# shehryar-malik/icrl

Hardware: AMD Instinct MI355X
Metric: env-steps/sec (ICRL outer loop, HCWithPos-v0) (higher is better)
Workload: dtype f32

## Files before the change

icrl_amd/csrc/rollout.hip:

```cpp
#include <stdio.h>
#include <stdlib.h>

#include "common.h"
#include "cost_fn.h"
#include "generic.h"

namespace icrl {

__global__ void policy_transpose_kernel(PolLayout L, const float* __restrict__ p, float* __restrict__ pt) {
  for (int i = blockIdx.x * blockDim.x + threadIdx.x; i < L.n; i += gridDim.x * blockDim.x) {
    int dst = i;
    for (int w = 0; w < 3; ++w) {
      if (i >= L.W1[w] && i < L.b1[w]) { int r = i - L.W1[w]; int j = r / L.O, k = r % L.O; dst = L.W1[w] + k * L.H1 + j; }
      if (i >= L.W2[w] && i < L.b2[w]) { int r = i - L.W2[w]; int j = r / L.H1, k = r % L.H1; dst = L.W2[w] + k * L.H2 + j; }
    }
    if (i >= L.Wa && i < L.ba) { int r = i - L.Wa; int a = r / L.H2, j = r % L.H2; dst = L.Wa + j * L.A + a; }
    pt[dst] = p[i];
  }
}

__global__ void costnet_transpose_kernel(CnLayout L, const float* __restrict__ p, float* __restrict__ pt) {
  for (int i = blockIdx.x * blockDim.x + threadIdx.x; i < L.n; i += gridDim.x * blockDim.x) {
    int dst = i;
    if (i >= L.W0 && i < L.b0) { int r = i - L.W0; int j = r / L.in, k = r % L.in; dst = L.W0 + k * L.H1 + j; }
    if (L.nh == 2 && i >= L.W1 && i < L.b1) { int r = i - L.W1; int j = r / L.H1, k = r % L.H1; dst = L.W1 + k * L.H2 + j; }
    pt[dst] = p[i];
  }
}

typedef float f32x4 __attribute__((ext_vector_type(4)));

struct ActShared {
  alignas(16) double s_old[MAX_OBS];
  alignas(16) double s_new[MAX_OBS];
  alignas(16) float x[MAX_OBS];
  alignas(16) float h[3][MAX_H];
  alignas(16) float g[3][MAX_H];
  alignas(16) float cx[MAX_CN_IN];
  alignas(16) float ch[2][MAX_H];
  float act_raw[MAX_ACT];
  float act_clip[MAX_ACT];
  float scal[4];
};

template <int OCT, int CIT>
struct WaveRegs {
  static constexpr int NA = 16 * (OCT > CIT ? OCT : CIT);
  union { float w1[NA]; float c0[NA]; };
  union { float w2[MAX_H]; float c1[MAX_H]; };
  float wh[MAX_H];
  union { float b1; float cb0; };
  union { float b2; float cb1; };
  union { float bh; float cbo; };
  union { float ls; float co; };
  float sd, lsd, i2v;
  int sel[(16 * (CIT > 0 ? CIT : 1) + WAVE - 1) / WAVE];
};
template <int OCT> using PolRegs = WaveRegs<OCT, 0>;
template <int CIT> using CnRegs = WaveRegs<0, CIT>;

template <int OCT, class Regs>
__device__ __forceinline__ void load_pol_regs(const PolLayout& L, const float* __restrict__ PT, Regs& R) {
  const int lane = threadIdx.x & 63;
  const int w = __builtin_amdgcn_readfirstlane(threadIdx.x >> 6);
  const int j1 = lane < L.H1 ? lane : 0, j2 = lane < L.H2 ? lane : 0;
#pragma unroll
  for (int k = 0; k < 16 * OCT; ++k) R.w1[k] = (w < 3 && k < L.O) ? PT[L.W1[w] + k * L.H1 + j1] : 0.f;
#pragma unroll
  for (int k = 0; k < MAX_H; ++k) R.w2[k] = (w < 3 && k < L.H1) ? PT[L.W2[w] + k * L.H2 + j2] : 0.f;
  R.b1 = w < 3 ? PT[L.b1[w] + j1] : 0.f;
  R.b2 = w < 3 ? PT[L.b2[w] + j2] : 0.f;
  R.bh = 0.f; R.ls = 0.f; R.sd = 1.f; R.lsd = 0.f; R.i2v = 2.f;
  if (w == 0) {
    const int a = lane < L.A ? lane : 0;
#pragma unroll
    for (int j = 0; j < MAX_H; ++j) R.wh[j] = j < L.H2 ? PT[L.Wa + j * L.A + a] : 0.f;
    R.bh = PT[L.ba + a];
    if (!L.discrete) R.ls = PT[L.log_std + a];
    R.sd = expf(R.ls); R.lsd = logf(R.sd); R.i2v = 2.f * (R.sd * R.sd);
  } else if (w < 3) {
#pragma unroll
    for (int j = 1; j < MAX_H; ++j) R.wh[j] = 0.f;
    R.wh[0] = PT[(w == 1 ? L.Wv : L.Wc) + j2];
    R.bh = PT[w == 1 ? L.bv : L.bc];
  }
}

template <int OCT, class Regs>
__device__ __forceinline__ void policy_forward_block(const PolLayout& L, const Regs& R, ActShared& sh,
                                                     const float* noise_row, int deterministic,
                                                     const float* alow, const float* ahigh,
                                                     const float* given = nullptr ) {
  const int lane = threadIdx.x & 63;
  const int w = __builtin_amdgcn_readfirstlane(threadIdx.x >> 6);
  if (w < 3) {
    f32x4 xs[4 * OCT];
#pragma unroll
    for (int i = 0; i < 4 * OCT; ++i) xs[i] = *reinterpret_cast<const f32x4*>(&sh.x[4 * i]);
    float acc = 0.f;
#pragma unroll
    for (int k = 0; k < 16 * OCT; ++k) acc = fmaf(R.w1[k], xs[k >> 2][k & 3], acc);
    sh.h[w][lane] = lane < L.H1 ? fast_tanh(acc + R.b1) : 0.f;
  }
  __syncthreads();
  if (w < 3) {
    f32x4 hs[MAX_H / 4];
#pragma unroll
    for (int i = 0; i < MAX_H / 4; ++i) hs[i] = *reinterpret_cast<const f32x4*>(&sh.h[w][4 * i]);
    float acc = 0.f;
#pragma unroll
    for (int k = 0; k < MAX_H; ++k) acc = fmaf(R.w2[k], hs[k >> 2][k & 3], acc);
    sh.g[w][lane] = lane < L.H2 ? fast_tanh(acc + R.b2) : 0.f;
  }
  __syncthreads();
  if (w == 0) {
    float mean = 0.f;
    {
      f32x4 gs[MAX_H / 4];
#pragma unroll
      for (int i = 0; i < MAX_H / 4; ++i) gs[i] = *reinterpret_cast<const f32x4*>(&sh.g[0][4 * i]);
      float acc = 0.f;
#pragma unroll
      for (int j = 0; j < MAX_H; ++j) acc = fmaf(R.wh[j], gs[j >> 2][j & 3], acc);
      mean = acc + R.bh;
    }
    if (!L.discrete) {
      float lp = 0.f, entl = 0.f;
      if (lane < L.A) {
        const float std = R.sd;
        float act = mean;
        if (given != nullptr) act = given[lane];
        else if (!deterministic) act = mean + noise_row[lane] * std;
        const float diff = act - mean;
        lp = -(diff * diff) / R.i2v - R.lsd - LOG_SQRT_2PI_F;
        entl = HALF_LOG_2PI_PLUS_HALF_F + R.lsd;
        sh.act_raw[lane] = act;
        float c = act;
        if (alow != nullptr && ahigh != nullptr) c = fminf(fmaxf(act, alow[lane]), ahigh[lane]);
        sh.act_clip[lane] = c;
      }
      lp = wave_sum_fast(lp);
      const float ent = wave_sum_fast(entl);
      if (lane == 0) { sh.scal[2] = lp; sh.scal[3] = ent; }
    } else {
      float m = wave_max(lane < L.A ? mean : -INFINITY);
      float e = lane < L.A ? expf(mean - m) : 0.f;
      float lse = m + logf(wave_sum(e));
      float logp = mean - lse;
      float p = lane < L.A ? expf(logp) : 0.f;
      float cdf = 0.f;
      int action = 0;
      if (given != nullptr) {
        action = (int)given[0];
      } else if (deterministic) {
        float best = wave_max(lane < L.A ? p : -1.f);
        unsigned long long ball = __ballot(lane < L.A && p == best);
        action = __ffsll((long long)ball) - 1;
      } else {
        const float u = noise_row[0];
        int cnt = 0;
        for (int a = 0; a < L.A; ++a) {
          cdf += __shfl(p, a, 64);
          cnt += (u >= cdf) ? 1 : 0;
        }
        action = cnt < L.A - 1 ? cnt : L.A - 1;
      }
      const float lp = __shfl(logp, action, 64);
      const float ent = -wave_sum(lane < L.A ? logp * p : 0.f);
      if (lane == 0) { sh.scal[2] = lp; sh.scal[3] = ent; sh.act_raw[0] = (float)action; sh.act_clip[0] = (float)action; }
    }
  } else if (w < 3) {
    float part = lane < L.H2 ? R.wh[0] * sh.g[w][lane] : 0.f;
    part = wave_sum_fast(part);
    if (lane == 0) sh.scal[w - 1] = part + R.bh;
  }
}

template <int CIT, class Regs>
__device__ __forceinline__ void load_cn_regs(const icrl_costnet_t& cn, const CnLayout& L, Regs& R) {
  const int lane = threadIdx.x & 63;
  const float* PT = cn.params_t;
  const int j1 = lane < L.H1 ? lane : 0, j2 = lane < L.H2 ? lane : 0;
#pragma unroll
  for (int k = 0; k < 16 * CIT; ++k) R.c0[k] = k < L.in ? PT[L.W0 + k * L.H1 + j1] : 0.f;
#pragma unroll
  for (int k = 0; k < MAX_H; ++k) R.c1[k] = (L.nh == 2 && k < L.H1) ? PT[L.W1 + k * L.H2 + j2] : 0.f;
  R.cb0 = PT[L.b0 + j1];
  R.cb1 = L.nh == 2 ? PT[L.b1 + j2] : 0.f;
  R.co = PT[L.Wo + j2];
  R.cbo = PT[L.bo];
#pragma unroll
  for (int i = 0; i < (16 * CIT + WAVE - 1) / WAVE; ++i) { const int idx = lane + i * WAVE; R.sel[i] = idx < L.in ? cn.select_dim[idx] : -1; }
}

template <int CIT, class Regs>
__device__ __forceinline__ float cost_forward_wave(const icrl_costnet_t& cn, const CnLayout& L, const Regs& R,
                                                   const double* obs_row, const float* acs_row, float* cx, float (*ch)[MAX_H],
                                                   int mode = 0 ) {
  const int lane = threadIdx.x & 63;
#pragma unroll
  for (int i = 0; i < (16 * CIT + WAVE - 1) / WAVE; ++i) {
    const int idx = lane + i * WAVE;
    const int sel = R.sel[i];
    float v = 0.f;
    if (sel >= 0) {
      if (sel < cn.obs_dim) {
        double o = obs_row[sel];
        if (cn.obs_mean != nullptr && cn.obs_var != nullptr) o = (o - cn.obs_mean[sel]) / sqrt(cn.obs_var[sel] + cn.eps);
        if (cn.clip_obs >= 0.0) o = fmin(fmax(o, -cn.clip_obs), cn.clip_obs);
        v = (float)o;
      } else {
        const int a = sel - cn.obs_dim;
        float x;
        if (cn.is_discrete) x = ((int)acs_row[0] == a) ? 1.f : 0.f;
        else x = acs_row[a];
        if (cn.action_low != nullptr && cn.action_high != nullptr) x = fminf(fmaxf(x, cn.action_low[a]), cn.action_high[a]);
        v = x;
      }
    }
    if (idx < 16 * CIT) cx[idx] = v;
  }
  __builtin_amdgcn_wave_barrier();
  __builtin_amdgcn_s_waitcnt(0xC07F);
  {
    f32x4 xs[4 * CIT];
#pragma unroll
    for (int i = 0; i < 4 * CIT; ++i) xs[i] = *reinterpret_cast<const f32x4*>(&cx[4 * i]);
    float acc = 0.f;
#pragma unroll
    for (int k = 0; k < 16 * CIT; ++k) acc = fmaf(R.c0[k], xs[k >> 2][k & 3], acc);
    ch[0][lane] = lane < L.H1 ? fmaxf(acc + R.cb0, 0.f) : 0.f;
  }
  __builtin_amdgcn_wave_barrier();
  __builtin_amdgcn_s_waitcnt(0xC07F);
  int last = 0;
  if (L.nh == 2) {
    f32x4 hs[MAX_H / 4];
#pragma unroll
    for (int i = 0; i < MAX_H / 4; ++i) hs[i] = *reinterpret_cast<const f32x4*>(&ch[0][4 * i]);
    float acc = 0.f;
#pragma unroll
    for (int k = 0; k < MAX_H; ++k) acc = fmaf(R.c1[k], hs[k >> 2][k & 3], acc);
    ch[1][lane] = lane < L.H2 ? fmaxf(acc + R.cb1, 0.f) : 0.f;
    __builtin_amdgcn_wave_barrier();
    __builtin_amdgcn_s_waitcnt(0xC07F);
    last = 1;
  }
  float part = lane < L.H2 ? R.co * ch[last][lane] : 0.f;
  const float z = wave_sum_fast(part) + R.cbo;
  const float zeta = 1.f / (1.f + expf(-z));
  if (mode == 1) return zeta;
  if (mode == 2) return logf(zeta + (float)cn.eps);
  return 1.f - zeta;
}

template <bool POINT = true>
__device__ __forceinline__ double env_reset_value(const icrl_env_t& e, uint32_t key, uint32_t ctr, int i) {
  if (POINT && e.reward_form >= 4) return e.reward_form == 12 ? (i == 0 ? 3.0 : 5.0) : 0.0;
  if (e.reward_form >= 2) return -1.0;
  return (unit_uniform(key, ctr, (uint32_t)(e.obs_dim + i)) - 0.5) * 0.2;
}

__device__ __forceinline__ void lap_grid_step_wave(const icrl_env_t& e, int n, const double* s_old, const float* act,
                                                   uint32_t& ctr_io, int& tep_io, double* s_new_lds, double& reward,
                                                   int& done) {
  const int lane = threadIdx.x & 63;
  const int pos_old = (int)llrint((s_old[0] + 1.0) * 20.0);
  const int ac = (int)act[0];
  int pos = pos_old, d = 0;
  double rew;
  if (ac == 0) {
    pos = pos_old + 1 == 40 ? 0 : pos_old + 1;
    rew = (pos % 10 == 5) ? 3.0 : 0.0;
  } else if (e.reward_form == 3) {
    rew = -1.0;
    d = 1;
  } else {
    pos = pos_old == 0 ? 39 : pos_old - 1;
    rew = (pos % 10 == 5) ? 3.0 : 0.0;
  }
  const int tep = tep_io + 1;
  if (tep >= e.max_steps) d = 1;
  if (d) pos = 0;
  const double v = ((double)pos * 2.0) / 40.0 - 1.0;
  tep_io = d ? 0 : tep;
  ctr_io = ctr_io + 1u;
  if (lane == 0) {
    e.s[n] = v;
    if (s_new_lds != nullptr) s_new_lds[0] = v;
    e.t_ep[n] = tep_io;
    e.step_count[n] = ctr_io;
  }
  reward = rew;
  done = d;
}

struct PointStep { double rew; int done; };
__device__ __forceinline__ int bridge_orientation(double p0, double p1, double q0, double q1, double r0, double r1) {
  const double val = ((q1 - p1) * (r0 - q0)) - ((q0 - p0) * (r1 - q1));
  return val == 0.0 ? 0 : (val > 0.0 ? 1 : -1);
}
__device__ __forceinline__ bool bridge_on_segment(double p0, double p1, double q0, double q1, double r0, double r1) {
  return r0 <= fmax(p0, q0) && r0 >= fmin(p0, q0) && r1 <= fmax(p1, q1) && r1 >= fmin(p1, q1);
}
__device__ __forceinline__ bool bridge_in_region(double sx, double sy, double nx, double ny, double ox, double oy, double w, double h) {
  const double x1 = ox + w, y1 = oy + h;
  if (sx > ox && sx < x1 && sy > oy && sy < y1) return true;
  if (nx > ox && nx < x1 && ny > oy && ny < y1) return true;
  bool hit = false;
#pragma unroll 1
  for (int b = 0; b < 4; ++b) {
    const double bp0 = b == 2 ? x1 : ox, bp1 = b == 3 ? y1 : oy;
    const double bq0 = b == 1 ? ox : x1, bq1 = b == 0 ? oy : y1;
    const int o1 = bridge_orientation(sx, sy, nx, ny, bp0, bp1);
    const int o2 = bridge_orientation(sx, sy, nx, ny, bq0, bq1);
    const int o3 = bridge_orientation(bp0, bp1, bq0, bq1, sx, sy);
    const int o4 = bridge_orientation(bp0, bp1, bq0, bq1, nx, ny);
    if (o1 != o2 && o3 != o4) hit = true;
    if (o1 == 0 && bridge_on_segment(sx, sy, nx, ny, bp0, bp1)) hit = true;
    if (o2 == 0 && bridge_on_segment(sx, sy, nx, ny, bq0, bq1)) hit = true;
    if (o3 == 0 && bridge_on_segment(bp0, bp1, bq0, bq1, sx, sy)) hit = true;
    if (o4 == 0 && bridge_on_segment(bp0, bp1, bq0, bq1, nx, ny)) hit = true;
  }
  return hit;
}
__device__ __noinline__ PointStep bridge_step_wave(int form, int max_steps, double* s_all, int32_t* t_ep_all, uint32_t* step_count_all,
                                                   int n, double x0, double y0, double ori0, float act0, float act1, uint32_t ctr_new,
                                                   int tep, double* s_new_lds) {
  const int lane = threadIdx.x & 63;
  const bool cont = form >= 13;
// ... 636 lines not shown
#pragma unroll
    for (int k = 0; k < 16; ++k) { const double d = va[k] - bm; va[k] = d * d; }
    __builtin_amdgcn_sched_barrier(0);
#pragma unroll
    for (int k = 0; k < 16; ++k) if (r0 + k < N) sq += va[k];
    load16(r0 + 32 < N ? r0 + 32 : 0, va);
#pragma unroll
    for (int k = 0; k < 16; ++k) { const double d = vb[k] - bm; vb[k] = d * d; }
    __builtin_amdgcn_sched_barrier(0);
#pragma unroll
    for (int k = 0; k < 16; ++k) if (r0 + 16 + k < N) sq += vb[k];
  }
  bv = sq / (double)N;
}

__device__ __forceinline__ void column_moments_contig(const double* col, int N, double& bm, double& bv) {
  double va[16], vb[16];
  double sum = 0.0;
  const int NF = N & ~31;
#pragma unroll
  for (int k = 0; k < 16; ++k) va[k] = col[k];
  int r0 = 0;
  for (; r0 < NF; r0 += 32) {
#pragma unroll
    for (int k = 0; k < 16; ++k) vb[k] = col[r0 + 16 + k];
    __builtin_amdgcn_sched_barrier(0);
#pragma unroll
    for (int k = 0; k < 16; ++k) sum += va[k];
#pragma unroll
    for (int k = 0; k < 16; ++k) va[k] = col[r0 + 32 + k];
    __builtin_amdgcn_sched_barrier(0);
#pragma unroll
    for (int k = 0; k < 16; ++k) sum += vb[k];
  }
  if (r0 < N) {
#pragma unroll
    for (int k = 0; k < 16; ++k) vb[k] = col[r0 + 16 + k];
#pragma unroll
    for (int k = 0; k < 16; ++k) if (r0 + k < N) sum += va[k];
#pragma unroll
    for (int k = 0; k < 16; ++k) if (r0 + 16 + k < N) sum += vb[k];
  }
  bm = sum / (double)N;
  double sq = 0.0;
#pragma unroll
  for (int k = 0; k < 16; ++k) va[k] = col[k];
  for (r0 = 0; r0 < NF; r0 += 32) {
#pragma unroll
    for (int k = 0; k < 16; ++k) vb[k] = col[r0 + 16 + k];
#pragma unroll
    for (int k = 0; k < 16; ++k) { const double d = va[k] - bm; va[k] = d * d; }
    __builtin_amdgcn_sched_barrier(0);
#pragma unroll
    for (int k = 0; k < 16; ++k) sq += va[k];
#pragma unroll
    for (int k = 0; k < 16; ++k) va[k] = col[r0 + 32 + k];
#pragma unroll
    for (int k = 0; k < 16; ++k) { const double d = vb[k] - bm; vb[k] = d * d; }
    __builtin_amdgcn_sched_barrier(0);
#pragma unroll
    for (int k = 0; k < 16; ++k) sq += vb[k];
  }
  if (r0 < N) {
#pragma unroll
    for (int k = 0; k < 16; ++k) vb[k] = col[r0 + 16 + k];
#pragma unroll
    for (int k = 0; k < 16; ++k) { const double d = va[k] - bm; va[k] = d * d; }
#pragma unroll
    for (int k = 0; k < 16; ++k) { const double d = vb[k] - bm; vb[k] = d * d; }
#pragma unroll
    for (int k = 0; k < 16; ++k) if (r0 + k < N) sq += va[k];
#pragma unroll
    for (int k = 0; k < 16; ++k) if (r0 + 16 + k < N) sq += vb[k];
  }
  bv = sq / (double)N;
}

__global__ void __launch_bounds__(1024) norm_step_small_kernel(NormStepArgs a) {
  __shared__ double chunk[NORM_CHUNK];
  __shared__ double vec[2][128], dev2[2][128];
  __shared__ double mean_s[MAX_OBS], var_s[MAX_OBS];
  __shared__ double dens[2];
  const int tid = threadIdx.x, nt = blockDim.x, lane = tid & 63, wv = tid >> 6;
  const int N = a.N, O = a.O;
  const icrl_norm_t& nm = a.nm;
  const bool has_cost = a.raw_cost != nullptr;
  for (int i = tid; i < N * O; i += nt) chunk[i] = a.raw_obs[i];
  if (tid < N) {
    double r = nm.ret[tid], c = has_cost ? nm.cost_ret[tid] : 0.0;
    if (nm.training) {
      r = r * nm.reward_gamma + a.raw_rew[tid];
      if (has_cost) c = c * nm.cost_gamma + (double)a.raw_cost[tid];
    }
    vec[0][tid] = r; vec[1][tid] = c;
  }
  double o_mean = 0.0, o_var = 1.0, o_cnt = 0.0;
  if (tid < O) { o_mean = nm.obs_mean[tid]; o_var = nm.obs_var[tid]; o_cnt = nm.obs_count[0]; }
  __syncthreads();
  if (nm.training) {
    if (tid < O) {
      double bm, bv;
      column_moments(chunk + tid, O, N, bm, bv);
      chan_merge(o_mean, o_var, o_cnt, bm, bv, (double)N);
      nm.obs_mean[tid] = o_mean; nm.obs_var[tid] = o_var;
      if (tid == 0) nm.obs_count[0] = (double)N + o_cnt;
    }
    if (wv == 15 || (wv == 14 && has_cost)) {
      const int v = wv == 15 ? 0 : 1;
      double* st = v == 0 ? nm.ret_stats : nm.cost_stats;
      const double bm = np_leaf_sum_wave(vec[v], N) / (double)N;
      for (int i = lane; i < N; i += 64) { const double d = vec[v][i] - bm; dev2[v][i] = d * d; }
      __builtin_amdgcn_wave_barrier();
      __builtin_amdgcn_s_waitcnt(0xC07F);
      const double bv = np_leaf_sum_wave(dev2[v], N) / (double)N;
      double m = st[0], var = st[1];
      const double cnt = st[2];
      chan_merge(m, var, cnt, bm, bv, (double)N);
      if (lane == 0) { st[0] = m; st[1] = var; st[2] = (double)N + cnt; }
      if (lane == 0) dens[v] = sqrt(var + nm.epsilon);
    }
  } else {
    if (tid == 0) { dens[0] = sqrt(nm.ret_stats[1] + nm.epsilon); dens[1] = sqrt(nm.cost_stats[1] + nm.epsilon); }
  }
  if (nm.training && !has_cost && tid == 0) dens[1] = sqrt(nm.cost_stats[1] + nm.epsilon);
  if (tid < O) { mean_s[tid] = o_mean; var_s[tid] = o_var; }
  __syncthreads();
  for (int idx = tid; idx < N * O; idx += nt) {
    const int j = idx % O;
    double o = chunk[idx];
    if (nm.norm_obs) o = fmin(fmax((o - mean_s[j]) / sqrt(var_s[j] + nm.epsilon), -nm.clip_obs), nm.clip_obs);
    if (a.obs_out) a.obs_out[idx] = o;
    if (a.obs_f32) a.obs_f32[idx] = (float)o;
  }
  if (tid < N) {
    const int n = tid;
    double r = a.raw_rew[n];
    if (nm.norm_reward) r = fmin(fmax(r / dens[0], -nm.clip_reward), nm.clip_reward);
    if (a.rew_out) a.rew_out[n] = r;
    if (a.rew_f32) a.rew_f32[n] = (float)r;
    const int d = a.dones[n];
    if (nm.training || d) nm.ret[n] = d ? 0.0 : vec[0][n];
    if (has_cost) {
      double c = (double)a.raw_cost[n];
      if (nm.norm_cost) c = fmin(fmax(c / dens[1], -nm.clip_cost), nm.clip_cost);
      if (a.cost_out) a.cost_out[n] = c;
      if (a.cost_f32) a.cost_f32[n] = (float)c;
      if (nm.training || d) nm.cost_ret[n] = d ? 0.0 : vec[1][n];
    }
    if (a.last_dones) a.last_dones[n] = (uint8_t)d;
  }
}

constexpr int NORM_MAX_N_TRACE = 1024;
__device__ unsigned long long g_rollout_prof[8];
__device__ unsigned long long g_rollout_prof_wide[16];
__device__ unsigned long long g_wide_trace[NORM_MAX_N_TRACE * 4];
__device__ __forceinline__ unsigned long long prof_now() {
  unsigned long long t;
  asm volatile("s_memtime %0\n\ts_waitcnt lgkmcnt(0)" : "=s"(t)::"memory");
  return t;
}

struct PersistArgs {
  ActStepArgs act;
  icrl_norm_t nm;
  int T;
  double* xch_obs;
  double* xch_rew;
  float* xch_cost;
  unsigned* xch_done;
  unsigned* counter;
  unsigned long long* xg;
  unsigned g_magic;
  int prof;
};

__device__ __forceinline__ void xstore(double* p, double v) {
  __hip_atomic_store(reinterpret_cast<unsigned long long*>(p), (unsigned long long)__double_as_longlong(v), __ATOMIC_RELAXED, __HIP_MEMORY_SCOPE_AGENT);
}
__device__ __forceinline__ void xstore(float* p, float v) {
  __hip_atomic_store(reinterpret_cast<unsigned*>(p), __float_as_uint(v), __ATOMIC_RELAXED, __HIP_MEMORY_SCOPE_AGENT);
}
__device__ __forceinline__ void xstore(unsigned* p, unsigned v) { __hip_atomic_store(p, v, __ATOMIC_RELAXED, __HIP_MEMORY_SCOPE_AGENT); }
__device__ __forceinline__ double xload(const double* p) {
  return __longlong_as_double((long long)__hip_atomic_load(reinterpret_cast<const unsigned long long*>(p), __ATOMIC_RELAXED, __HIP_MEMORY_SCOPE_AGENT));
}
__device__ __forceinline__ float xload(const float* p) {
  return __uint_as_float(__hip_atomic_load(reinterpret_cast<const unsigned*>(p), __ATOMIC_RELAXED, __HIP_MEMORY_SCOPE_AGENT));
}
__device__ __forceinline__ unsigned xload(const unsigned* p) { return __hip_atomic_load(p, __ATOMIC_RELAXED, __HIP_MEMORY_SCOPE_AGENT); }
__device__ __forceinline__ void gstore(unsigned long long* p, unsigned tag, unsigned payload) {
  __hip_atomic_store(p, ((unsigned long long)tag << 32) | (unsigned long long)payload, __ATOMIC_RELAXED, __HIP_MEMORY_SCOPE_AGENT);
}
__device__ __forceinline__ unsigned long long gload(const unsigned long long* p) {
  return __hip_atomic_load(p, __ATOMIC_RELAXED, __HIP_MEMORY_SCOPE_AGENT);
}

__device__ __forceinline__ void grid_barrier(unsigned* flags, int N, int n, unsigned value, int& spin_limit) {
  asm volatile("s_waitcnt vmcnt(0)" ::: "memory");
  __syncthreads();
  if (threadIdx.x < 64) {
    const int lane = threadIdx.x;
    if (lane == 0) xstore(flags + n, value);
    int spins = 0;
    bool ok = false;
    while (spins < spin_limit && !ok) {
      const unsigned v0 = lane < N ? xload(flags + lane) : value;
      const unsigned v1 = lane + 64 < N ? xload(flags + lane + 64) : value;
      ok = __all(v0 >= value && v1 >= value);
      ++spins;
    }
    if (!ok) spin_limit = 1;
  }
  __syncthreads();
}

constexpr int GRAN_MAX = 12;
constexpr int REC_MAX = GRAN_MAX / 2;

static inline size_t persist_dyn_lds(int N, int O, int A) { return ((size_t)O * (size_t)(N + 64) + (size_t)O * (size_t)A) * sizeof(double); }

template <int OCT, int CIT, bool GRAN, bool PROF = false, bool MON = false, bool POINT = true, bool DISC = false, bool SDE = false, bool REGION = false>
__device__ __forceinline__ void rollout_persistent_body(const PersistArgs& p, const SdeArgs& sd = SdeArgs()) {
  extern __shared__ __attribute__((aligned(16))) double dyn_lds[];
  __shared__ ActShared sh;
  double* const chunk = dyn_lds;
  double* const Bl = dyn_lds + p.act.pl.O * (p.act.env.n_envs + 64);
  __shared__ double vec[2][128], dev2[2][128], ret_s[128], cret_s[128], rawr_s[128];
  __shared__ float rawc_s[128];
  __shared__ double dens[2];
  __shared__ float noise_s[MAX_ACT], alow_s[MAX_ACT], ahigh_s[MAX_ACT];
  __shared__ int done_s[128];
  __shared__ int last_done_s;
  const ActStepArgs& a = p.act;
  REGION_TABLE(a, (int)threadIdx.x, 256)
  icrl_norm_t nm = p.nm; globalize(nm);
  icrl_buffer_t buf = a.buf; globalize(buf);
  icrl_agent_t ag = a.ag; globalize(ag);
  icrl_costnet_t cnet = a.cn; globalize(cnet);
  unsigned long long* const xg_all = as_global(p.xg);
  const float* const noise_g = as_global(a.noise);
  double* const raw_plane = MON ? as_global(a.raw_plane) : nullptr;
  WaveRegs<OCT, CIT> R;
  WaveRegs<OCT, CIT>& C = R;
  load_pol_regs<OCT>(a.pl, a.PT, R);
  if constexpr (CIT > 0) { if (threadIdx.x >= 192 && a.has_cn) load_cn_regs<CIT>(a.cn, a.cl, C); }
  const icrl_cost_fn_t cf = a.cf;
  const int n = blockIdx.x;
  const int tid = threadIdx.x, lane = tid & 63;
  const int w = __builtin_amdgcn_readfirstlane(tid >> 6);
  const int O = a.pl.O, A = a.pl.A, N = a.env.n_envs, T = p.T;
  const int AS = buf.act_store;
  const int NA = a.pl.discrete ? 1 : A;
  const int NP = N + 64;
  const int G = 2 * O + 4;
  const int R16 = O + 2;
  typedef unsigned int rec_u4 __attribute__((ext_vector_type(4)));
  const __amdgpu_buffer_rsrc_t xrs = __builtin_amdgcn_make_buffer_rsrc(xg_all, 0, 2 * N * G * 8, 0x00020000);
  auto rstore = [&](int byte_off, rec_u4 v) { __builtin_amdgcn_raw_buffer_store_b128(v, xrs, byte_off, 0, 16); };
  auto rload = [&](int byte_off) -> rec_u4 { return __builtin_amdgcn_raw_buffer_load_b128(xrs, byte_off, 0, 16); };
  for (int i = tid; i < O * NP; i += 256) chunk[i] = 0.0;
  constexpr int SDE_REGS = MAX_H * MAX_ACT / 256;
  double* const e2_s = SDE ? Bl + O * a.env.act_dim : nullptr;
  float* const E_s = SDE ? reinterpret_cast<float*>(e2_s + MAX_H * A) : nullptr;
  const float* const expl_n = SDE ? as_global(sd.expl) + (size_t)n * (size_t)sd.env_stride : nullptr;
  float e_reg[SDE_REGS];
  if constexpr (SDE) {
    const float* const ls_g = as_global(sd.ls);
    for (int i = tid; i < MAX_H * A; i += 256) e2_s[i] = exp(2. * (double)ls_g[i]);
#pragma unroll
    for (int k = 0; k < SDE_REGS; ++k) { const int i = k * 256 + tid; e_reg[k] = i < MAX_H * A ? expl_n[i] : 0.f; }
  }
  const bool has_cost = a.has_cn != 0;
  const uint32_t e_key = a.env.key[n];
  uint32_t e_ctr = a.env.step_count[n];
  int e_tep = a.env.t_ep[n];
  icrl_env_t env = a.env; globalize(env);
  for (int i = tid; i < O * a.env.act_dim; i += 256) Bl[i] = a.env.B[i];
  env.B = Bl;
  const bool has_box = a.alow != nullptr && a.ahigh != nullptr;
  if (tid < MAX_ACT) { alow_s[tid] = (has_box && tid < A) ? a.alow[tid] : 0.f; ahigh_s[tid] = (has_box && tid < A) ? a.ahigh[tid] : 0.f; }
  for (int i = tid; i < MAX_OBS; i += 256) {
    sh.x[i] = i < O ? (float)ag.last_obs[(size_t)n * O + i] : 0.f;
    if (i < O) sh.s_old[i] = a.env.s[(size_t)n * O + i];
  }
  if (tid < N) { ret_s[tid] = nm.ret[tid]; cret_s[tid] = nm.cost_ret[tid]; }
  if (tid == 0) last_done_s = ag.last_dones[n];
  double o_mean = 0.0, o_var = 1.0, o_cnt = 0.0, o_last = 0.0;
  if (tid < O) { o_mean = nm.obs_mean[tid]; o_var = nm.obs_var[tid]; o_cnt = nm.obs_count[0]; o_last = ag.last_obs[(size_t)n * O + tid]; }
  double st_m = 0.0, st_v = 1.0, st_c = 0.0;
  if (w == 3) { st_m = nm.ret_stats[0]; st_v = nm.ret_stats[1]; st_c = nm.ret_stats[2]; }
  if (w == 2) { st_m = nm.cost_stats[0]; st_v = nm.cost_stats[1]; st_c = nm.cost_stats[2]; }
  float noise_reg = (!SDE && tid < NA) ? noise_g[(size_t)n * NA + tid] : 0.f;
  double fin_rew = 0.0; float fin_cost = 0.f; int fin_done = 0;
  unsigned long long pc0 = 0, pc1 = 0, pc2 = 0, pc3 = 0, pc4 = 0, pc5 = 0, pc_rounds = 0, tl = PROF ? prof_now() : 0ull;
  int spin_limit = 1 << 22;
  for (int t = 0; t < T; ++t) {
    const int par = t & 1;
    const size_t tn = (size_t)t * N + n;
    const unsigned gtag = (unsigned)(t + 1);
    if (!SDE && tid < NA) {
      noise_s[tid] = noise_reg;
      if (t + 1 < T) noise_reg = noise_g[((size_t)(t + 1) * N + n) * NA + tid];
    }
    if constexpr (SDE) {
      const int sf = sd.sample_freq;
      if (t == 0 || (sf > 0 && t % sf == 0)) {
#pragma unroll
        for (int k = 0; k < SDE_REGS; ++k) { const int i = k * 256 + tid; if (i < MAX_H * A) E_s[i] = e_reg[k]; }
      }
      if (t + 1 < T && sf > 0 && (t + 1) % sf == 0) {
        const float* const nxt = expl_n + (size_t)((t + 1) / sf) * (size_t)sd.draw_stride;
#pragma unroll
        for (int k = 0; k < SDE_REGS; ++k) { const int i = k * 256 + tid; e_reg[k] = i < MAX_H * A ? nxt[i] : 0.f; }
      }
    }
    __syncthreads();
    if constexpr (SDE) {
      policy_forward_block<OCT>(a.pl, R, sh, nullptr, 1, nullptr, nullptr);
      if (w == 0) sde_head_wave(sh, A, a.pl.H2, E_s, [&](int i) { return e2_s[i]; }, has_box ? alow_s : nullptr, has_box ? ahigh_s : nullptr);
    } else {
      policy_forward_block<OCT>(a.pl, R, sh, noise_s, 0, has_box ? alow_s : nullptr, has_box ? ahigh_s : nullptr);
    }
    __syncthreads();
    if (w == 0) {
      double rew; int done;
      env_step_wave<POINT>(env, n, sh.s_old, sh.act_clip, e_key, e_ctr, e_tep, sh.s_new, rew, done);
      float* nob = buf.new_orig_observations + tn * O;
      if (GRAN) {
        const int rec0 = ((par * N + n) * R16) * 16;
        for (int i = lane; i < O; i += WAVE) {
          const double v = sh.s_new[i];
          nob[i] = (float)v;
          const unsigned long long bits = (unsigned long long)__double_as_longlong(v);
          rstore(rec0 + 16 * i, rec_u4{gtag, (unsigned)bits, (unsigned)(bits >> 32), gtag});
        }
        if (lane == 0) {
          const unsigned long long bits = (unsigned long long)__double_as_longlong(rew);
          rstore(rec0 + 16 * O, rec_u4{gtag, (unsigned)bits, (unsigned)(bits >> 32), gtag | (done ? 0x80000000u : 0u)});
        }
      } else {
        double* xo = as_global(p.xch_obs) + ((size_t)par * N + n) * O;
        for (int i = lane; i < O; i += WAVE) { const double v = sh.s_new[i]; nob[i] = (float)v; xstore(xo + i, v); }
        if (lane == 0) { xstore(as_global(p.xch_rew) + par * N + n, rew); xstore(as_global(p.xch_done) + par * N + n, (unsigned)done); }
      }
    } else if (w == 3) {
      float cost = 0.f;
      if constexpr (REGION) cost = cost_region_wave(rtab, a.cr.n_clauses, a.cr.combine, sh.s_old, sh.act_clip, O);
      else if constexpr (CIT == 0) cost = cost_fn_wave(cf, sh.s_old, sh.act_clip);
      else if (a.has_cn) cost = cost_forward_wave<CIT>(cnet, a.cl, C, sh.s_old, sh.act_clip, sh.cx, sh.ch, DISC ? 1 : 0);
      if (lane == 0) {
        if (GRAN) rstore(((par * N + n) * R16 + O + 1) * 16, rec_u4{gtag, __float_as_uint(cost), 0u, gtag});
        else xstore(as_global(p.xch_cost) + par * N + n, cost);
        buf.orig_costs[tn] = cost;
      }
    } else if (w == 2) {
      float* ob = buf.observations + tn * O;
      float* oob = buf.orig_observations + tn * O;
      for (int i = lane; i < O; i += WAVE) { ob[i] = sh.x[i]; oob[i] = (float)sh.s_old[i]; }
      if (lane < AS) buf.actions[tn * AS + lane] = sh.act_raw[lane];
      if (lane < A && !a.pl.discrete) ag.act_clipped[(size_t)n * A + lane] = sh.act_clip[lane];
      if (lane == 0) {
        buf.dones[tn] = (float)last_done_s;
        buf.reward_values[tn] = sh.scal[0];
        buf.cost_values[tn] = sh.scal[1];
        buf.log_probs[tn] = sh.scal[2];
        ag.last_v_r[n] = sh.scal[0];
        ag.last_v_c[n] = sh.scal[1];
      }
    }
    if (PROF) { const unsigned long long tn_ = prof_now(); pc0 += tn_ - tl; tl = tn_; }
    if (PROF && t == T / 2 && lane == 0) g_wide_trace[4 * n + w] = __builtin_amdgcn_s_memrealtime();
    if (GRAN) {
      const int rbase = par * N * R16 * 16;
      const int total = N * R16;
      rec_u4 g[REC_MAX];
#pragma unroll
      for (int k = 0; k < REC_MAX; ++k) g[k] = (k * 256 + tid < total) ? rload(rbase + (k * 256 + tid) * 16) : rec_u4{gtag, 0u, 0u, gtag};
      bool ok = false;
      int rounds = 0;
      for (int spins = 0; spins < spin_limit && !ok; ++spins) {
        ok = true;
#pragma unroll
        for (int k = 0; k < REC_MAX; ++k)
          if (g[k][0] != gtag || (g[k][3] & 0x7fffffffu) != gtag) { g[k] = rload(rbase + (k * 256 + tid) * 16); ok = false; }
        ++rounds;
      }
      if (PROF && tid == 0) { pc_rounds += (unsigned long long)rounds; }
      if (!ok) spin_limit = 1;
#pragma unroll
      for (int k = 0; k < REC_MAX; ++k) {
        const int idx = k * 256 + tid;
        if (idx < total) {
          unsigned rr = __umulhi((unsigned)idx, p.g_magic);
          int slot = idx - (int)rr * R16;
          if (slot >= R16) { slot -= R16; ++rr; }
          const double v = __longlong_as_double((long long)(((unsigned long long)g[k][2] << 32) | (unsigned long long)g[k][1]));
          if (slot < O) chunk[slot * NP + (int)rr] = v;
          else if (slot == O) { rawr_s[rr] = v; done_s[rr] = (int)(g[k][3] >> 31); }
          else rawc_s[rr] = has_cost ? __uint_as_float(g[k][1]) : 0.f;
        }
      }
      __syncthreads();
    } else {
      grid_barrier(as_global(p.counter), N, n, (unsigned)(t + 1), spin_limit);
    }
    if (PROF) { const unsigned long long tn_ = prof_now(); pc1 += tn_ - tl; tl = tn_; }
    {
      if (!GRAN) {
        const double* xo = as_global(p.xch_obs) + (size_t)par * N * O;
        for (int i = tid; i < N * O; i += 256) { const int rr = i / O, j = i - rr * O; chunk[j * NP + rr] = xload(xo + i); }
      }
      if (tid < N) {
        if (!GRAN) {
          rawr_s[tid] = xload(as_global(p.xch_rew) + par * N + tid);
          rawc_s[tid] = has_cost ? xload(as_global(p.xch_cost) + par * N + tid) : 0.f;
          done_s[tid] = (int)xload(as_global(p.xch_done) + par * N + tid);
        }
        const double rr = rawr_s[tid];
        const float rc = rawc_s[tid];
        double r = ret_s[tid], c = has_cost ? cret_s[tid] : 0.0;
        if (nm.training) {
          r = r * nm.reward_gamma + rr;
          if (has_cost) c = c * nm.cost_gamma + (double)rc;
        }
        vec[0][tid] = r; vec[1][tid] = c;
      }
    }
    __syncthreads();
    if (PROF) { const unsigned long long tn_ = prof_now(); pc3 += tn_ - tl; tl = tn_; }
    if (nm.training) {
      if (tid < O) {
        double bm, bv;
        column_moments_contig(chunk + tid * NP, N, bm, bv);
        chan_merge(o_mean, o_var, o_cnt, bm, bv, (double)N);
        o_cnt = (double)N + o_cnt;
      }
      if (w == 3 || (w == 2 && has_cost)) {
        const int v = w == 3 ? 0 : 1;
        const double bm = np_leaf_sum_wave(vec[v], N) / (double)N;
        for (int i = lane; i < N; i += 64) { const double d = vec[v][i] - bm; dev2[v][i] = d * d; }
        __builtin_amdgcn_wave_barrier();
        __builtin_amdgcn_s_waitcnt(0xC07F);
        const double bv = np_leaf_sum_wave(dev2[v], N) / (double)N;
        chan_merge(st_m, st_v, st_c, bm, bv, (double)N);
        st_c = (double)N + st_c;
      }
    }
    if (lane == 0 && w == 3) dens[0] = sqrt(st_v + nm.epsilon);
    if (lane == 0 && w == 2) dens[1] = sqrt(st_v + nm.epsilon);
    if (PROF) { const unsigned long long tn_ = prof_now(); pc4 += tn_ - tl; tl = tn_; }
    if (tid < O) {
      double o = chunk[tid * NP + n];
      if (nm.norm_obs) o = fmin(fmax((o - o_mean) / sqrt(o_var + nm.epsilon), -nm.clip_obs), nm.clip_obs);
      o_last = o;
      sh.x[tid] = (float)o;
      buf.new_observations[tn * O + tid] = (float)o;
      sh.s_old[tid] = sh.s_new[tid];
    }
    __syncthreads();
    if (PROF) { const unsigned long long tn_ = prof_now(); pc5 += tn_ - tl; tl = tn_; }
    if (tid < N) {
      const int d = done_s[tid];
      if (nm.training || d) { ret_s[tid] = d ? 0.0 : vec[0][tid]; if (has_cost) cret_s[tid] = d ? 0.0 : vec[1][tid]; }
    }
    if (tid == 0) {
      double r = rawr_s[n];
      fin_rew = r; fin_cost = rawc_s[n]; fin_done = done_s[n];
      if (nm.norm_reward) r = fmin(fmax(r / dens[0], -nm.clip_reward), nm.clip_reward);
      buf.rewards[tn] = (float)r;
      if (has_cost) {
        double c = (double)rawc_s[n];
        if (nm.norm_cost) c = fmin(fmax(c / dens[1], -nm.clip_cost), nm.clip_cost);
        buf.costs[tn] = (float)c;
      }
      last_done_s = done_s[n];
      if (MON) raw_plane[tn] = fin_rew;
    }
    if (PROF) { const unsigned long long tn_ = prof_now(); pc2 += tn_ - tl; tl = tn_; }
  }
  if (PROF && n == 0 && tid == 0) { g_rollout_prof[0] = pc0; g_rollout_prof[1] = pc1; g_rollout_prof[2] = pc2; g_rollout_prof[3] = (unsigned long long)T; g_rollout_prof[4] = pc3; g_rollout_prof[5] = pc4; g_rollout_prof[6] = pc5; g_rollout_prof[7] = pc_rounds; }
  if (spin_limit == 1 && ag.status != nullptr && (tid & 63) == 0) atomicOr(ag.status, 1);
  __syncthreads();
  if (tid < O) ag.last_obs[(size_t)n * O + tid] = o_last;
  if (tid == 0) {
    ag.last_dones[n] = (uint8_t)last_done_s;
    ag.raw_rew[n] = fin_rew; ag.dones[n] = (uint8_t)fin_done;
    if (has_cost) ag.raw_cost[n] = fin_cost;
  }
  if (n == 0) {
    if (tid < O) { nm.obs_mean[tid] = o_mean; nm.obs_var[tid] = o_var; }
    if (tid == 0) nm.obs_count[0] = o_cnt;
    if (lane == 0 && w == 3) { nm.ret_stats[0] = st_m; nm.ret_stats[1] = st_v; nm.ret_stats[2] = st_c; }
    if (lane == 0 && w == 2 && has_cost) { nm.cost_stats[0] = st_m; nm.cost_stats[1] = st_v; nm.cost_stats[2] = st_c; }
    if (tid < N) { nm.ret[tid] = ret_s[tid]; if (has_cost) nm.cost_ret[tid] = cret_s[tid]; }
  }
}

struct GenRolloutArgs {
  PersistArgs p;
  GenNet net;
  const float* P;
};
template <int OCT, int CIT, bool MON, bool DISC = false>
__device__ __forceinline__ void rollout_generic_body(const GenRolloutArgs& ga) {
  constexpr bool GRAN = true;
  const PersistArgs& p = ga.p;
  const GenNet& net = ga.net;
  __shared__ float gact[GEN_MAX_ROW];
  extern __shared__ __attribute__((aligned(16))) double dyn_lds[];
  __shared__ ActShared sh;
  double* const chunk = dyn_lds;
  double* const Bl = dyn_lds + p.act.pl.O * (p.act.env.n_envs + 64);
  __shared__ double vec[2][128], dev2[2][128], ret_s[128], cret_s[128], rawr_s[128];
  __shared__ float rawc_s[128];
  __shared__ double dens[2];
  __shared__ float noise_s[MAX_ACT], alow_s[MAX_ACT], ahigh_s[MAX_ACT];
  __shared__ int done_s[128];
  __shared__ int last_done_s;
  const ActStepArgs& a = p.act;
  icrl_norm_t nm = p.nm; globalize(nm);
  icrl_buffer_t buf = a.buf; globalize(buf);
  icrl_agent_t ag = a.ag; globalize(ag);
  icrl_costnet_t cnet = a.cn; globalize(cnet);
  unsigned long long* const xg_all = as_global(p.xg);
  const float* const noise_g = as_global(a.noise);
  double* const raw_plane = MON ? as_global(a.raw_plane) : nullptr;
  WaveRegs<OCT, CIT> R;
  WaveRegs<OCT, CIT>& C = R;
  if constexpr (CIT > 0) { if ((threadIdx.x >> 6) == 3 && a.has_cn) load_cn_regs<CIT>(a.cn, a.cl, C); }
  const icrl_cost_fn_t cf = a.cf;
  const int n = blockIdx.x;
  const int tid = threadIdx.x, lane = tid & 63;
  const int ctid = tid < 256 ? tid : (1 << 28);
  const float* const Pn = as_global(ga.P);
  const float* const PTn = as_global(a.PT);
  const int w = __builtin_amdgcn_readfirstlane(tid >> 6);
  const int O = a.pl.O, A = a.pl.A, N = a.env.n_envs, T = p.T;
  const int AS = buf.act_store;
  const int NA = a.pl.discrete ? 1 : A;
  const int NP = N + 64;
  const int G = 2 * O + 4;
  const int R16 = O + 2;
  typedef unsigned int rec_u4 __attribute__((ext_vector_type(4)));
  const __amdgpu_buffer_rsrc_t xrs = __builtin_amdgcn_make_buffer_rsrc(xg_all, 0, 2 * N * G * 8, 0x00020000);
  auto rstore = [&](int byte_off, rec_u4 v) { __builtin_amdgcn_raw_buffer_store_b128(v, xrs, byte_off, 0, 16); };
  auto rload = [&](int byte_off) -> rec_u4 { return __builtin_amdgcn_raw_buffer_load_b128(xrs, byte_off, 0, 16); };
  for (int i = ctid; i < O * NP; i += 256) chunk[i] = 0.0;
  const bool has_cost = a.has_cn != 0;
  const uint32_t e_key = a.env.key[n];
  uint32_t e_ctr = a.env.step_count[n];
  int e_tep = a.env.t_ep[n];
  icrl_env_t env = a.env; globalize(env);
  for (int i = ctid; i < O * a.env.act_dim; i += 256) Bl[i] = a.env.B[i];
  env.B = Bl;
  const bool has_box = a.alow != nullptr && a.ahigh != nullptr;
  if (tid < MAX_ACT) { alow_s[tid] = (has_box && tid < A) ? a.alow[tid] : 0.f; ahigh_s[tid] = (has_box && tid < A) ? a.ahigh[tid] : 0.f; }
  for (int i = ctid; i < MAX_OBS; i += 256) {
    sh.x[i] = i < O ? (float)ag.last_obs[(size_t)n * O + i] : 0.f;
    if (i < O) sh.s_old[i] = a.env.s[(size_t)n * O + i];
  }
  if (tid < N) { ret_s[tid] = nm.ret[tid]; cret_s[tid] = nm.cost_ret[tid]; }
  if (tid == 0) last_done_s = ag.last_dones[n];
  double o_mean = 0.0, o_var = 1.0, o_cnt = 0.0, o_last = 0.0;
  if (tid < O) { o_mean = nm.obs_mean[tid]; o_var = nm.obs_var[tid]; o_cnt = nm.obs_count[0]; o_last = ag.last_obs[(size_t)n * O + tid]; }
  double st_m = 0.0, st_v = 1.0, st_c = 0.0;
  if (w == 3) { st_m = nm.ret_stats[0]; st_v = nm.ret_stats[1]; st_c = nm.ret_stats[2]; }
  if (w == 2) { st_m = nm.cost_stats[0]; st_v = nm.cost_stats[1]; st_c = nm.cost_stats[2]; }
  float noise_reg = (tid < NA) ? noise_g[(size_t)n * NA + tid] : 0.f;
  double fin_rew = 0.0; float fin_cost = 0.f; int fin_done = 0;
  unsigned long long pc0 = 0, pc1 = 0, pc2 = 0, pc3 = 0, pc4 = 0, pc5 = 0, pc_rounds = 0, tl = p.prof ? prof_now() : 0ull;
  int spin_limit = 1 << 22;
  for (int t = 0; t < T; ++t) {
    const int par = t & 1;
    const size_t tn = (size_t)t * N + n;
    const unsigned gtag = (unsigned)(t + 1);
    if (tid < NA) {
      noise_s[tid] = noise_reg;
      if (t + 1 < T) noise_reg = noise_g[((size_t)(t + 1) * N + n) * NA + tid];
    }
    __syncthreads();
    gen_mlp_forward_quads(net, PTn, sh.x, gact, w, lane);
    if (tid == 0) {
      float lp, ent;
      gen_policy_head(net, Pn, gact + net.layer[net.head[0]].act_off, noise_s, 0, has_box ? alow_s : nullptr, has_box ? ahigh_s : nullptr, nullptr,
                      sh.act_raw, sh.act_clip, lp, ent);
      sh.scal[0] = gact[net.layer[net.head[1]].act_off]; sh.scal[1] = gact[net.layer[net.head[2]].act_off]; sh.scal[2] = lp;
    }
    __syncthreads();
    if (w == 0) {
      double rew; int done;
      env_step_wave(env, n, sh.s_old, sh.act_clip, e_key, e_ctr, e_tep, sh.s_new, rew, done);
      float* nob = buf.new_orig_observations + tn * O;
      if (GRAN) {
        const int rec0 = ((par * N + n) * R16) * 16;
        for (int i = lane; i < O; i += WAVE) {
          const double v = sh.s_new[i];
          nob[i] = (float)v;
          const unsigned long long bits = (unsigned long long)__double_as_longlong(v);
          rstore(rec0 + 16 * i, rec_u4{gtag, (unsigned)bits, (unsigned)(bits >> 32), gtag});
        }
        if (lane == 0) {
          const unsigned long long bits = (unsigned long long)__double_as_longlong(rew);
          rstore(rec0 + 16 * O, rec_u4{gtag, (unsigned)bits, (unsigned)(bits >> 32), gtag | (done ? 0x80000000u : 0u)});
        }
      } else {
        double* xo = as_global(p.xch_obs) + ((size_t)par * N + n) * O;
        for (int i = lane; i < O; i += WAVE) { const double v = sh.s_new[i]; nob[i] = (float)v; xstore(xo + i, v); }
        if (lane == 0) { xstore(as_global(p.xch_rew) + par * N + n, rew); xstore(as_global(p.xch_done) + par * N + n, (unsigned)done); }
      }
    } else if (w == 3) {
      float cost = 0.f;
      if constexpr (CIT == 0) cost = cost_fn_wave(cf, sh.s_old, sh.act_clip);
      else if (a.has_cn) cost = cost_forward_wave<CIT>(cnet, a.cl, C, sh.s_old, sh.act_clip, sh.cx, sh.ch, DISC ? 1 : 0);
      if (lane == 0) {
        if (GRAN) rstore(((par * N + n) * R16 + O + 1) * 16, rec_u4{gtag, __float_as_uint(cost), 0u, gtag});
        else xstore(as_global(p.xch_cost) + par * N + n, cost);
        buf.orig_costs[tn] = cost;
      }
    } else if (w == 2) {
      float* ob = buf.observations + tn * O;
      float* oob = buf.orig_observations + tn * O;
      for (int i = lane; i < O; i += WAVE) { ob[i] = sh.x[i]; oob[i] = (float)sh.s_old[i]; }
      if (lane < AS) buf.actions[tn * AS + lane] = sh.act_raw[lane];
      if (lane < A && !a.pl.discrete) ag.act_clipped[(size_t)n * A + lane] = sh.act_clip[lane];
      if (lane == 0) {
        buf.dones[tn] = (float)last_done_s;
        buf.reward_values[tn] = sh.scal[0];
        buf.cost_values[tn] = sh.scal[1];
        buf.log_probs[tn] = sh.scal[2];
        ag.last_v_r[n] = sh.scal[0];
        ag.last_v_c[n] = sh.scal[1];
      }
    }
    if (p.prof) { const unsigned long long tn_ = prof_now(); pc0 += tn_ - tl; tl = tn_; }
    if (p.prof && t == T / 2 && lane == 0) g_wide_trace[4 * n + w] = __builtin_amdgcn_s_memrealtime();
    if (GRAN) {
      const int rbase = par * N * R16 * 16;
// ... 3571 lines not shown
```

Baseline: 984,000.

## Replace block barriers in policy forward with per-wave chain and wave-local LDS ordering

Each of the three policy waves now computes its own forward chain (shared hidden layer copy per wave) and orders its LDS traffic with wave barriers, so the pre-forward and intra-forward block __syncthreads are removed for the non-SDE path. Log-prob is computed by the env wave after publishing, value heads are written directly by their waves, and in GRAN mode the return-vector update and done reset are spread over waves 2/3 instead of tid<N, dropping one block barrier. Tail bookkeeping moves to thread 192 to offload wave 0, and profiling marks are added. This risks LDS ordering bugs, since waves now rely only on wave-level ordering between writes and later reads.

```diff
diff --git a/icrl_amd/csrc/rollout.hip b/icrl_amd/csrc/rollout.hip
--- a/icrl_amd/csrc/rollout.hip
+++ b/icrl_amd/csrc/rollout.hip
@@ -176,6 +176,88 @@
   }
 }
 
+__device__ __forceinline__ void wave_lds_order() {
+  __builtin_amdgcn_s_waitcnt(0xC07F);
+  __builtin_amdgcn_wave_barrier();
+}
+template <int OCT, class Regs>
+__device__ __forceinline__ float policy_forward_chain(const PolLayout& L, const Regs& R, ActShared& sh, const float* noise_row,
+                                                      const float* alow, const float* ahigh) {
+  const int lane = threadIdx.x & 63;
+  const int w = __builtin_amdgcn_readfirstlane(threadIdx.x >> 6);
+  if (w >= 3) return 0.f;
+  {
+    f32x4 xs[4 * OCT];
+#pragma unroll
+    for (int i = 0; i < 4 * OCT; ++i) xs[i] = *reinterpret_cast<const f32x4*>(&sh.x[4 * i]);
+    float acc = 0.f;
+#pragma unroll
+    for (int k = 0; k < 16 * OCT; ++k) acc = fmaf(R.w1[k], xs[k >> 2][k & 3], acc);
+    sh.h[w][lane] = lane < L.H1 ? fast_tanh(acc + R.b1) : 0.f;
+  }
+  wave_lds_order();
+  {
+    f32x4 hs[MAX_H / 4];
+#pragma unroll
+    for (int i = 0; i < MAX_H / 4; ++i) hs[i] = *reinterpret_cast<const f32x4*>(&sh.h[w][4 * i]);
+    float acc = 0.f;
+#pragma unroll
+    for (int k = 0; k < MAX_H; ++k) acc = fmaf(R.w2[k], hs[k >> 2][k & 3], acc);
+    sh.g[w][lane] = lane < L.H2 ? fast_tanh(acc + R.b2) : 0.f;
+  }
+  wave_lds_order();
+  if (w != 0) {
+    float part = lane < L.H2 ? R.wh[0] * sh.g[w][lane] : 0.f;
+    part = wave_sum_fast(part);
+    return part + R.bh;
+  }
+  float mean = 0.f;
+  {
+    f32x4 gs[MAX_H / 4];
+#pragma unroll
+    for (int i = 0; i < MAX_H / 4; ++i) gs[i] = *reinterpret_cast<const f32x4*>(&sh.g[0][4 * i]);
+    float acc = 0.f;
+#pragma unroll
+    for (int j = 0; j < MAX_H; ++j) acc = fmaf(R.wh[j], gs[j >> 2][j & 3], acc);
+    mean = acc + R.bh;
+  }
+  if (!L.discrete) {
+    float diff = 0.f;
+    if (lane < L.A) {
+      const float act = mean + noise_row[lane] * R.sd;
+      diff = act - mean;
+      sh.act_raw[lane] = act;
+      float c = act;
+      if (alow != nullptr && ahigh != nullptr) c = fminf(fmaxf(act, alow[lane]), ahigh[lane]);
+      sh.act_clip[lane] = c;
+    }
+    return diff;
+  }
+  float m = wave_max(lane < L.A ? mean : -INFINITY);
+  float e = lane < L.A ? expf(mean - m) : 0.f;
+  float lse = m + logf(wave_sum(e));
+  float logp = mean - lse;
+  float p = lane < L.A ? expf(logp) : 0.f;
+  float cdf = 0.f;
+  const float u = noise_row[0];
+  int cnt = 0;
+  for (int a = 0; a < L.A; ++a) {
+    cdf += __shfl(p, a, 64);
+    cnt += (u >= cdf) ? 1 : 0;
+  }
+  const int action = cnt < L.A - 1 ? cnt : L.A - 1;
+  if (lane == 0) { sh.act_raw[0] = (float)action; sh.act_clip[0] = (float)action; }
+  return __shfl(logp, action, 64);
+}
+template <class Regs>
+__device__ __forceinline__ float chain_log_prob(const PolLayout& L, const Regs& R, float head) {
+  if (L.discrete) return head;
+  const int lane = threadIdx.x & 63;
+  float lp = 0.f;
+  if (lane < L.A) lp = -(head * head) / R.i2v - R.lsd - LOG_SQRT_2PI_F;
+  return wave_sum_fast(lp);
+}
+
 template <int CIT, class Regs>
 __device__ __forceinline__ void load_cn_regs(const icrl_costnet_t& cn, const CnLayout& L, Regs& R) {
   const int lane = threadIdx.x & 63;
@@ -1118,6 +1200,7 @@
 }
 
 constexpr int NORM_MAX_N_TRACE = 1024;
+constexpr int CHAIN_TRACE_BASE = 4 * 128;
 __device__ unsigned long long g_rollout_prof[8];
 __device__ unsigned long long g_rollout_prof_wide[16];
 __device__ unsigned long long g_wide_trace[NORM_MAX_N_TRACE * 4];
@@ -1260,11 +1343,17 @@
   float noise_reg = (!SDE && tid < NA) ? noise_g[(size_t)n * NA + tid] : 0.f;
   double fin_rew = 0.0; float fin_cost = 0.f; int fin_done = 0;
   unsigned long long pc0 = 0, pc1 = 0, pc2 = 0, pc3 = 0, pc4 = 0, pc5 = 0, pc_rounds = 0, tl = PROF ? prof_now() : 0ull;
+  enum { CH_FWD, CH_HANDOFF, CH_ENV, CH_PUBLISH, CH_AFTER_PUB, CH_POLL, CH_SCATTER, CH_VEC, CH_COLUMNS, CH_MERGE, CH_NORMALISE, CH_REST, CH_PUB_AT, CH_N };
+  unsigned long long fc[CH_N] = {0}, fl = 0, f0 = 0;
+  auto mark = [&](int k) { if (PROF) { const unsigned long long now = prof_now(); fc[k] += now - fl; fl = now; } };
+  constexpr int TAIL = 192;
   int spin_limit = 1 << 22;
+  if constexpr (!SDE) __syncthreads();
   for (int t = 0; t < T; ++t) {
     const int par = t & 1;
     const size_t tn = (size_t)t * N + n;
     const unsigned gtag = (unsigned)(t + 1);
+    if (PROF) { fl = prof_now(); f0 = fl; }
     if (!SDE && tid < NA) {
       noise_s[tid] = noise_reg;
       if (t + 1 < T) noise_reg = noise_g[((size_t)(t + 1) * N + n) * NA + tid];
@@ -1281,17 +1370,23 @@
         for (int k = 0; k < SDE_REGS; ++k) { const int i = k * 256 + tid; e_reg[k] = i < MAX_H * A ? nxt[i] : 0.f; }
       }
     }
-    __syncthreads();
+    if constexpr (SDE) __syncthreads();
+    else wave_lds_order();
+    float head = 0.f;
     if constexpr (SDE) {
       policy_forward_block<OCT>(a.pl, R, sh, nullptr, 1, nullptr, nullptr);
       if (w == 0) sde_head_wave(sh, A, a.pl.H2, E_s, [&](int i) { return e2_s[i]; }, has_box ? alow_s : nullptr, has_box ? ahigh_s : nullptr);
     } else {
-      policy_forward_block<OCT>(a.pl, R, sh, noise_s, 0, has_box ? alow_s : nullptr, has_box ? ahigh_s : nullptr);
-    }
+      head = policy_forward_chain<OCT>(a.pl, R, sh, noise_s, has_box ? alow_s : nullptr, has_box ? ahigh_s : nullptr);
+    }
+    mark(CH_FWD);
     __syncthreads();
+    mark(CH_HANDOFF);
+    if (SDE && w < 3) head = sh.scal[w == 0 ? 2 : w - 1];
     if (w == 0) {
       double rew; int done;
       env_step_wave<POINT>(env, n, sh.s_old, sh.act_clip, e_key, e_ctr, e_tep, sh.s_new, rew, done);
+      mark(CH_ENV);
       float* nob = buf.new_orig_observations + tn * O;
       if (GRAN) {
         const int rec0 = ((par * N + n) * R16) * 16;
@@ -1310,6 +1405,10 @@
         for (int i = lane; i < O; i += WAVE) { const double v = sh.s_new[i]; nob[i] = (float)v; xstore(xo + i, v); }
         if (lane == 0) { xstore(as_global(p.xch_rew) + par * N + n, rew); xstore(as_global(p.xch_done) + par * N + n, (unsigned)done); }
       }
+      if (PROF) { mark(CH_PUBLISH); fc[CH_PUB_AT] += fl - f0; }
+      const float lp = SDE ? head : chain_log_prob(a.pl, R, head);
+      if (lane == 0) buf.log_probs[tn] = lp;
+      mark(CH_AFTER_PUB);
     } else if (w == 3) {
       float cost = 0.f;
       if constexpr (REGION) cost = cost_region_wave(rtab, a.cr.n_clauses, a.cr.combine, sh.s_old, sh.act_clip, O);
@@ -1328,12 +1427,11 @@
       if (lane < A && !a.pl.discrete) ag.act_clipped[(size_t)n * A + lane] = sh.act_clip[lane];
       if (lane == 0) {
         buf.dones[tn] = (float)last_done_s;
-        buf.reward_values[tn] = sh.scal[0];
-        buf.cost_values[tn] = sh.scal[1];
-        buf.log_probs[tn] = sh.scal[2];
-        ag.last_v_r[n] = sh.scal[0];
-        ag.last_v_c[n] = sh.scal[1];
-      }
+        buf.cost_values[tn] = head;
+        ag.last_v_c[n] = head;
+      }
+    } else {
+      if (lane == 0) { buf.reward_values[tn] = head; ag.last_v_r[n] = head; }
     }
     if (PROF) { const unsigned long long tn_ = prof_now(); pc0 += tn_ - tl; tl = tn_; }
     if (PROF && t == T / 2 && lane == 0) g_wide_trace[4 * n + w] = __builtin_amdgcn_s_memrealtime();
@@ -1353,6 +1451,7 @@
         ++rounds;
       }
       if (PROF && tid == 0) { pc_rounds += (unsigned long long)rounds; }
+      mark(CH_POLL);
       if (!ok) spin_limit = 1;
 #pragma unroll
       for (int k = 0; k < REC_MAX; ++k) {
@@ -1372,6 +1471,25 @@
       grid_barrier(as_global(p.counter), N, n, (unsigned)(t + 1), spin_limit);
     }
     if (PROF) { const unsigned long long tn_ = prof_now(); pc1 += tn_ - tl; tl = tn_; }
+    mark(CH_SCATTER);
+    if constexpr (GRAN) {
+      if (w == 3) {
+        for (int i = lane; i < N; i += 64) {
+          const double rr = rawr_s[i];
+          double r = ret_s[i];
+          if (nm.training) r = r * nm.reward_gamma + rr;
+          vec[0][i] = r;
+        }
+      } else if (w == 2) {
+        for (int i = lane; i < N; i += 64) {
+          const float rc = rawc_s[i];
+          double c = has_cost ? cret_s[i] : 0.0;
+          if (nm.training && has_cost) c = c * nm.cost_gamma + (double)rc;
+          vec[1][i] = c;
+        }
+      }
+      if (w >= 2) wave_lds_order();
+    } else
     {
       if (!GRAN) {
         const double* xo = as_global(p.xch_obs) + (size_t)par * N * O;
@@ -1392,15 +1510,18 @@
         }
         vec[0][tid] = r; vec[1][tid] = c;
       }
-    }
-    __syncthreads();
+      __syncthreads();
+    }
     if (PROF) { const unsigned long long tn_ = prof_now(); pc3 += tn_ - tl; tl = tn_; }
+    mark(CH_VEC);
     if (nm.training) {
       if (tid < O) {
         double bm, bv;
         column_moments_contig(chunk + tid * NP, N, bm, bv);
+        mark(CH_COLUMNS);
         chan_merge(o_mean, o_var, o_cnt, bm, bv, (double)N);
         o_cnt = (double)N + o_cnt;
+        mark(CH_MERGE);
       }
       if (w == 3 || (w == 2 && has_cost)) {
         const int v = w == 3 ? 0 : 1;
@@ -1426,11 +1547,19 @@
     }
     __syncthreads();
     if (PROF) { const unsigned long long tn_ = prof_now(); pc5 += tn_ - tl; tl = tn_; }
+    mark(CH_NORMALISE);
+    if (GRAN) {
+      if (w == 3) {
+        for (int i = lane; i < N; i += 64) { const int d = done_s[i]; if (nm.training || d) ret_s[i] = d ? 0.0 : vec[0][i]; }
+      } else if (w == 2 && has_cost) {
+        for (int i = lane; i < N; i += 64) { const int d = done_s[i]; if (nm.training || d) cret_s[i] = d ? 0.0 : vec[1][i]; }
+      }
+    } else
     if (tid < N) {
       const int d = done_s[tid];
       if (nm.training || d) { ret_s[tid] = d ? 0.0 : vec[0][tid]; if (has_cost) cret_s[tid] = d ? 0.0 : vec[1][tid]; }
     }
-    if (tid == 0) {
+    if (tid == TAIL) {
       double r = rawr_s[n];
       fin_rew = r; fin_cost = rawc_s[n]; fin_done = done_s[n];
       if (nm.norm_reward) r = fmin(fmax(r / dens[0], -nm.clip_reward), nm.clip_reward);
@@ -1444,12 +1573,17 @@
       if (MON) raw_plane[tn] = fin_rew;
     }
     if (PROF) { const unsigned long long tn_ = prof_now(); pc2 += tn_ - tl; tl = tn_; }
+    mark(CH_REST);
   }
   if (PROF && n == 0 && tid == 0) { g_rollout_prof[0] = pc0; g_rollout_prof[1] = pc1; g_rollout_prof[2] = pc2; g_rollout_prof[3] = (unsigned long long)T; g_rollout_prof[4] = pc3; g_rollout_prof[5] = pc4; g_rollout_prof[6] = pc5; g_rollout_prof[7] = pc_rounds; }
+  if (PROF && n == 0 && tid == 0) {
+#pragma unroll
+    for (int k = 0; k < CH_N; ++k) g_wide_trace[CHAIN_TRACE_BASE + k] = fc[k];
+  }
   if (spin_limit == 1 && ag.status != nullptr && (tid & 63) == 0) atomicOr(ag.status, 1);
   __syncthreads();
   if (tid < O) ag.last_obs[(size_t)n * O + tid] = o_last;
-  if (tid == 0) {
+  if (tid == TAIL) {
     ag.last_dones[n] = (uint8_t)last_done_s;
     ag.raw_rew[n] = fin_rew; ag.dones[n] = (uint8_t)fin_done;
     if (has_cost) ag.raw_cost[n] = fin_cost;
```

Measured after the change: 995,200 (median of 6 runs). 1.1% higher.
